# Ankur-Deka/Emergent-Multiagent-Strategies

Measured on AMD Instinct MI355X. Metric: env-steps/sec FortAttack 3v3, 4096 parallel envs per GPU, higher is better.
Workload: dtype f64

## Files before the change

emergent-multiagent-strategies_amd/csrc/fa_collect.hip:

```cpp
#include "fa_device.h"

#define FA_GAE_CHUNK 16
struct FaGaeChunk { float r[FA_GAE_CHUNK], v[FA_GAE_CHUNK], m[FA_GAE_CHUNK]; uint8_t d[FA_GAE_CHUNK]; };
__global__ __launch_bounds__(64) void fa_gae_kernel(const float *__restrict__ rewards,
                                                    const float *__restrict__ value_preds,
                                                    const float *__restrict__ masks,
                                                    float *__restrict__ returns,
                                                    const uint8_t *__restrict__ done, int T, int E,
                                                    int N, float g32, float gt32) {
    const long long EN = (long long)E * N;
    const long long col = (long long)blockIdx.x * blockDim.x + threadIdx.x;
    if (col >= EN) return;
    const int e = (int)(col / N);
    float gae = 0.0f;
    float v_next = value_preds[(long long)T * EN + col];
    float m_next = masks[(long long)T * EN + col];
    auto load = [&](FaGaeChunk &c, int t0) {
#pragma unroll
        for (int k = 0; k < FA_GAE_CHUNK; ++k) {
            const int t = t0 - k;
            const long long o = (long long)(t >= 0 ? t : 0) * EN + col;
            c.r[k] = rewards[o];
            c.v[k] = value_preds[o];
            c.m[k] = masks[o];
            c.d[k] = done[(long long)(t > 0 ? t - 1 : 0) * E + e];
        }
    };
    auto scan = [&](const FaGaeChunk &c, int t0) {
#pragma unroll
        for (int k = 0; k < FA_GAE_CHUNK; ++k) {
            const int t = t0 - k;
            if (t >= 0) {
                const float delta = c.r[k] + g32 * v_next * m_next - c.v[k];
                const float g = delta + gt32 * m_next * gae;
                if ((t > 0) & (c.d[k] != 0)) {
                    gae = 0.0f;
                } else {
                    gae = g;
                    returns[(long long)t * EN + col] = g + c.v[k];
                }
                v_next = c.v[k];
                m_next = c.m[k];
            }
        }
    };
    FaGaeChunk ca, cb;
    load(ca, T - 1);
    for (int t0 = T - 1; t0 >= 0; t0 -= 2 * FA_GAE_CHUNK) {
        load(cb, t0 - FA_GAE_CHUNK);
        scan(ca, t0);
        load(ca, t0 - 2 * FA_GAE_CHUNK);
        scan(cb, t0 - FA_GAE_CHUNK);
    }
}

#define FA_GAEC_CHUNK 32
__global__ __launch_bounds__(256) void fa_gae_coop_kernel(const float *__restrict__ rewards,
                                                          const float *__restrict__ value_preds,
                                                          const float *__restrict__ masks,
                                                          float *__restrict__ returns,
                                                          const uint8_t *__restrict__ done, int T, int E,
                                                          int N, float g32, float gt32) {
    __shared__ float s_r[2][FA_GAEC_CHUNK][64], s_v[2][FA_GAEC_CHUNK][64], s_m[2][FA_GAEC_CHUNK][64];
    __shared__ uint8_t s_d[2][FA_GAEC_CHUNK][64];
    const long long EN = (long long)E * N;
    const int lane = threadIdx.x & 63, wave = threadIdx.x >> 6;
    const long long colv = (long long)blockIdx.x * 64 + lane;
    const bool valid = colv < EN;
    const long long col = valid ? colv : EN - 1;
    const int e = (int)(col / N);
    const int nc = (T + FA_GAEC_CHUNK - 1) / FA_GAEC_CHUNK;
    auto load_chunk = [&](int c) {
        const int t0 = T - 1 - c * FA_GAEC_CHUNK, b = c & 1;
        if (wave == 3) {
            float x[FA_GAEC_CHUNK];
            uint8_t d[FA_GAEC_CHUNK];
#pragma unroll
            for (int k = 0; k < FA_GAEC_CHUNK; ++k) {
                const int t = t0 - k;
                x[k] = masks[(long long)(t >= 0 ? t : 0) * EN + col];
                d[k] = done[(long long)(t > 0 ? t - 1 : 0) * E + e];
            }
#pragma unroll
            for (int k = 0; k < FA_GAEC_CHUNK; ++k) { s_m[b][k][lane] = x[k]; s_d[b][k][lane] = d[k]; }
        } else {
            const float *src = wave == 1 ? rewards : value_preds;
            float x[FA_GAEC_CHUNK];
#pragma unroll
            for (int k = 0; k < FA_GAEC_CHUNK; ++k) {
                const int t = t0 - k;
                x[k] = src[(long long)(t >= 0 ? t : 0) * EN + col];
            }
            float(*dst)[64] = wave == 1 ? s_r[b] : s_v[b];
#pragma unroll
            for (int k = 0; k < FA_GAEC_CHUNK; ++k) dst[k][lane] = x[k];
        }
    };
    float gae = 0.0f, v_next = 0.0f, m_next = 0.0f;
    if (wave == 0) {
        v_next = value_preds[(long long)T * EN + col];
        m_next = masks[(long long)T * EN + col];
    } else {
        load_chunk(0);
    }
    __syncthreads();
    for (int c = 0; c < nc; ++c) {
        if (wave != 0) {
            if (c + 1 < nc) load_chunk(c + 1);
        } else {
            const int t0 = T - 1 - c * FA_GAEC_CHUNK, b = c & 1;
            float r[FA_GAEC_CHUNK], v[FA_GAEC_CHUNK], m[FA_GAEC_CHUNK];
            uint8_t d[FA_GAEC_CHUNK];
#pragma unroll
            for (int k = 0; k < FA_GAEC_CHUNK; ++k) {
                r[k] = s_r[b][k][lane]; v[k] = s_v[b][k][lane]; m[k] = s_m[b][k][lane]; d[k] = s_d[b][k][lane];
            }
#pragma unroll
            for (int k = 0; k < FA_GAEC_CHUNK; ++k) {
                const int t = t0 - k;
                if (t >= 0) {
                    const float delta = r[k] + g32 * v_next * m_next - v[k];
                    const float g = delta + gt32 * m_next * gae;
                    if ((t > 0) & (d[k] != 0)) {
                        gae = 0.0f;
                    } else {
                        gae = g;
                        if (valid) returns[(long long)t * EN + col] = g + v[k];
                    }
                    v_next = v[k];
                    m_next = m[k];
                }
            }
        }
        __syncthreads();
    }
}


#define FA_GAEC_GATHER 4
#define FA_GAEC_BARRIER() asm volatile("s_waitcnt lgkmcnt(0)\n\ts_barrier" ::: "memory")
__device__ __forceinline__ float fa_gae_pivot(const float *__restrict__ rewards, const float *__restrict__ value_preds,
                                              const float *__restrict__ masks, int T, long long EN, int i, float g32) {
    const long long o = (long long)(T - 1) * EN + i, o1 = (long long)T * EN + i;
    const float vp = value_preds[o];
    const float delta = rewards[o] + g32 * value_preds[o1] * masks[o1] - vp;
    return (delta + vp) - vp;
}

__global__ __launch_bounds__(256, 2) void fa_gae_mom_kernel(const float *__restrict__ rewards,
                                                             const float *__restrict__ value_preds,
                                                             const float *__restrict__ masks, float *__restrict__ returns,
                                                             const uint8_t *__restrict__ done, int T, int E, int N, float g32,
                                                             float gt32, double *__restrict__ partial) {
    __shared__ float s_x[3][2][FA_GAEC_CHUNK][64];
    __shared__ uint8_t s_d[2][FA_GAEC_CHUNK][64];
    __shared__ double s_sq[2][64];
    const long long EN = (long long)E * N;
    const int lane = threadIdx.x & 63, wave = __builtin_amdgcn_readfirstlane(threadIdx.x >> 6);
    const long long colv = (long long)blockIdx.x * 64 + lane;
    const bool valid = colv < EN;
    const long long col = valid ? colv : EN - 1;
    const int e = (int)(col / N);
    const int nc = (T + FA_GAEC_CHUNK - 1) / FA_GAEC_CHUNK;
    const unsigned rowb = (unsigned)EN * 4u;
    const unsigned coff = (unsigned)col * 4u;
    const float *src = wave == 1 ? rewards : (wave == 2 ? value_preds : masks);
    const __amdgpu_buffer_rsrc_t rs_src =
        __builtin_amdgcn_make_buffer_rsrc(const_cast<float *>(src), 0, (int)((unsigned)(T + 1) * rowb), 0x00020000);
    const __amdgpu_buffer_rsrc_t rs_ret = __builtin_amdgcn_make_buffer_rsrc(returns, 0, (int)((unsigned)(T + 1) * rowb), 0x00020000);
    const __amdgpu_buffer_rsrc_t rs_val =
        __builtin_amdgcn_make_buffer_rsrc(const_cast<float *>(value_preds), 0, (int)((unsigned)(T + 1) * rowb), 0x00020000);
    const __amdgpu_buffer_rsrc_t rs_done =
        __builtin_amdgcn_make_buffer_rsrc(const_cast<uint8_t *>(done), 0, (int)((unsigned)T * (unsigned)E), 0x00020000);
    auto ldf = [&](const __amdgpu_buffer_rsrc_t &rs, unsigned voff, unsigned soff) -> float {
        return __builtin_bit_cast(float, __builtin_amdgcn_raw_buffer_load_b32(rs, (int)voff, __builtin_amdgcn_readfirstlane((int)soff), 0));
    };
    struct Chunk { float x[FA_GAEC_CHUNK]; uint8_t d[FA_GAEC_CHUNK]; };
    auto issue = [&](Chunk &q, int c) {
        const int t0 = T - 1 - c * FA_GAEC_CHUNK;
#pragma unroll
        for (int k = 0; k < FA_GAEC_CHUNK; ++k) {
            const int t = t0 - k;
            q.x[k] = ldf(rs_src, coff, (unsigned)(t >= 0 ? t : 0) * rowb);
        }
        if (wave == 3) {
#pragma unroll
            for (int k = 0; k < FA_GAEC_CHUNK; ++k) {
                const int t = t0 - k;
                q.d[k] = __builtin_amdgcn_raw_buffer_load_b8(rs_done, e, __builtin_amdgcn_readfirstlane((int)((unsigned)(t > 0 ? t - 1 : 0) * (unsigned)E)), 0);
            }
        }
    };
    auto stash = [&](const Chunk &q, int c) {
        float(*dst)[64] = s_x[wave - 1][c & 1];
#pragma unroll
        for (int k = 0; k < FA_GAEC_CHUNK; ++k) dst[k][lane] = q.x[k];
        if (wave == 3) {
#pragma unroll
            for (int k = 0; k < FA_GAEC_CHUNK; ++k) s_d[c & 1][k][lane] = q.d[k];
        }
    };
    if (wave != 0) {
        Chunk q;
        issue(q, 0);
        stash(q, 0);
        FA_GAEC_BARRIER();
        for (int c = 0; c < nc; ++c) {
            if (c + 1 < nc) {
                issue(q, c + 1);
                stash(q, c + 1);
            }
            FA_GAEC_BARRIER();
        }
    } else {
        float gae = 0.0f;
        float v_next = value_preds[(long long)T * EN + col];
        float m_next = masks[(long long)T * EN + col];
        double accS[2] = {0.0, 0.0}, accQ[2] = {0.0, 0.0};
        const double piv = (double)fa_gae_pivot(rewards, value_preds, masks, T, EN, (int)(col % N), g32);
        auto add_stale = [&](float o, float v) {
            const double dd = (double)(o - v) - piv;
            accS[0] += dd;
            accQ[0] = __fma_rn(dd, dd, accQ[0]);
        };
        float go[FA_GAEC_GATHER], gv[FA_GAEC_GATHER];
        unsigned gmask = 0u;
#pragma unroll
        for (int j = 0; j < FA_GAEC_GATHER; ++j) { go[j] = 0.0f; gv[j] = 0.0f; }
        FA_GAEC_BARRIER();
        auto scan_chunk = [&](int c) {
            const int t0 = T - 1 - c * FA_GAEC_CHUNK, b = c & 1;
#pragma unroll
            for (int j = 0; j < FA_GAEC_GATHER; ++j)
                if ((gmask >> j) & 1u) add_stale(go[j], gv[j]);
            float r[FA_GAEC_CHUNK], v[FA_GAEC_CHUNK], m[FA_GAEC_CHUNK];
            uint8_t d[FA_GAEC_CHUNK];
#pragma unroll
            for (int k = 0; k < FA_GAEC_CHUNK; ++k) {
                r[k] = s_x[0][b][k][lane]; v[k] = s_x[1][b][k][lane]; m[k] = s_x[2][b][k][lane]; d[k] = s_d[b][k][lane];
            }
            unsigned stale = 0u;
#pragma unroll
            for (int k = 0; k < FA_GAEC_CHUNK; ++k) {
                const int t = t0 - k;
                if (t >= 0) {
                    const float delta = r[k] + g32 * v_next * m_next - v[k];
                    const float g = delta + gt32 * m_next * gae;
                    if ((t > 0) & (d[k] != 0)) {
                        gae = 0.0f;
                        stale |= 1u << k;
                    } else {
                        gae = g;
                        const float ret = g + v[k];
                        if (valid) __builtin_amdgcn_raw_buffer_store_b32(__builtin_bit_cast(unsigned, ret), rs_ret, (int)coff, __builtin_amdgcn_readfirstlane((int)((unsigned)t * rowb)), 0);
                        const double dd = (double)(ret - v[k]) - piv;
                        accS[k & 1] += dd;
                        accQ[k & 1] = __fma_rn(dd, dd, accQ[k & 1]);
                    }
                    v_next = v[k];
                    m_next = m[k];
                }
            }
            {
                unsigned rem = stale;
                gmask = 0u;
#pragma unroll
                for (int j = 0; j < FA_GAEC_GATHER; ++j) {
                    const int k = rem ? __builtin_ctz(rem) : 0;
                    gmask |= (rem ? 1u : 0u) << j;
                    rem &= rem - 1u;
                    const unsigned o = (unsigned)(t0 - k) * rowb + coff;
                    go[j] = ldf(rs_ret, o, 0u);
                    gv[j] = ldf(rs_val, o, 0u);
                }
                while (__builtin_amdgcn_ballot_w64(rem != 0u) != 0ull) {
                    const bool has = rem != 0u;
                    const int k = has ? __builtin_ctz(rem) : 0;
                    rem &= rem - 1u;
                    const unsigned o = (unsigned)(t0 - k) * rowb + coff;
                    const float o_ = ldf(rs_ret, o, 0u), v_ = ldf(rs_val, o, 0u);
                    if (has) add_stale(o_, v_);
                }
            }
        };
        for (int c = 0; c < nc; ++c) {
            scan_chunk(c);
            FA_GAEC_BARRIER();
        }
#pragma unroll
        for (int j = 0; j < FA_GAEC_GATHER; ++j)
            if ((gmask >> j) & 1u) add_stale(go[j], gv[j]);
        s_sq[0][lane] = valid ? accS[0] + accS[1] : 0.0;
        s_sq[1][lane] = valid ? accQ[0] + accQ[1] : 0.0;
    }
    {
        __syncthreads();
        if ((int)threadIdx.x < 2 * N) {
            const int i = threadIdx.x >> 1, cmp = threadIdx.x & 1;
            const int first = (int)(((long long)blockIdx.x * 64) % N);
            double acc = 0.0;
            for (int l = (i - first + N) % N; l < 64; l += N) acc += s_sq[cmp][l];
            partial[((long long)blockIdx.x * N + i) * 2 + cmp] = acc;
        }
    }
}

#define FA_GAEM_FOLD 8
__device__ __forceinline__ void fa_gae_mom_fold(const double *__restrict__ partial, int nblocks, int N, int i, int lane,
                                                double n_rows, double piv, double &mean, double &m2) {
    const double2 *p2 = reinterpret_cast<const double2 *>(partial);
    double2 p[FA_GAEM_FOLD];
#pragma unroll
    for (int k = 0; k < FA_GAEM_FOLD; ++k) {
        const int b = lane + 64 * k;
        p[k] = p2[(long long)(b < nblocks ? b : 0) * N + i];
    }
    double s = 0.0, q = 0.0;
#pragma unroll
    for (int k = 0; k < FA_GAEM_FOLD; ++k) {
        const bool in = lane + 64 * k < nblocks;
        s += in ? p[k].x : 0.0;
        q += in ? p[k].y : 0.0;
    }
#pragma unroll
    for (int off = 32; off > 0; off >>= 1) { s += __shfl_down(s, off, 64); q += __shfl_down(q, off, 64); }
    s = __shfl(s, 0, 64);
    q = __shfl(q, 0, 64);
    mean = piv + s / n_rows;
    m2 = q - s * (s / n_rows);
}

__global__ void fa_gae_mom_final_kernel(const double *__restrict__ partial, int nblocks, int N,
                                        const float *__restrict__ rewards, const float *__restrict__ value_preds,
                                        const float *__restrict__ masks, int T, long long EN, float g32, double n_rows,
                                        double *__restrict__ moments_out, double *__restrict__ mean_out,
                                        double *__restrict__ std_out) {
    const int i = threadIdx.x >> 6, lane = threadIdx.x & 63;
    if (i >= N) return;
    const double piv = (double)fa_gae_pivot(rewards, value_preds, masks, T, EN, i, g32);
    double mean, m2;
    fa_gae_mom_fold(partial, nblocks, N, i, lane, n_rows, piv, mean, m2);
    if (lane == 0) {
        if (moments_out) { moments_out[i * 3 + 0] = n_rows; moments_out[i * 3 + 1] = mean; moments_out[i * 3 + 2] = m2; }
        if (mean_out) mean_out[i] = mean;
        if (std_out) std_out[i] = sqrt(m2 / (n_rows - 1.0));
    }
}

__global__ __launch_bounds__(512) void fa_gae_mom_norm_kernel(const double *__restrict__ partial, int nblocks, int N,
                                                              const float *__restrict__ rewards,
                                                              const float *__restrict__ value_preds,
                                                              const float *__restrict__ masks,
                                                              const float *__restrict__ returns, int T, long long EN, float g32,
                                                              double n_rows, long long total, float *__restrict__ out,
                                                              double *__restrict__ moments_out, double *__restrict__ mean_out,
                                                              double *__restrict__ std_out, int piv_from_returns,
                                                              const double *__restrict__ gathered, int W) {
    __shared__ float s_mean[FA_MAX_AGENTS_DEV], s_den[FA_MAX_AGENTS_DEV];
    const int lane = threadIdx.x & 63, wave = threadIdx.x >> 6;
    const long long stride = (long long)gridDim.x * blockDim.x;
    const long long gid = (long long)blockIdx.x * blockDim.x + threadIdx.x;
    const long long quads = total / 4;
    const bool vec = (((uintptr_t)returns | (uintptr_t)value_preds | (uintptr_t)out) & 15) == 0;
    const float4 *r4 = reinterpret_cast<const float4 *>(returns), *v4 = reinterpret_cast<const float4 *>(value_preds);
    float4 ra = make_float4(0.f, 0.f, 0.f, 0.f), va = ra, rb = ra, vb = ra;
    if (vec && gid < quads) {
        const long long q1 = gid + stride;
        ra = r4[gid]; va = v4[gid];
        rb = r4[q1 < quads ? q1 : gid]; vb = v4[q1 < quads ? q1 : gid];
    }
    if (gathered) {
        if ((int)threadIdx.x < N) {
            const int i = threadIdx.x;
            double n = 0.0, mean = 0.0, m2 = 0.0;
            for (int r = 0; r < W; ++r) {
                const double *g = gathered + ((long long)r * N + i) * 3;
                const double nr = g[0], mr = g[1], m2r = g[2];
                if (nr <= 0.0) continue;
                const double nn = n + nr, delta = mr - mean;
                mean += delta * (nr / nn);
                m2 += m2r + delta * delta * (n * nr / nn);
                n = nn;
            }
            const double sd = sqrt(m2 / (n - 1.0));
            s_mean[i] = (float)mean;
            s_den[i] = (float)sd + 1e-5f;
            if (blockIdx.x == 0) {
                if (mean_out) mean_out[i] = mean;
                if (std_out) std_out[i] = sd;
            }
        }
    } else
    for (int i = wave; i < N; i += 8) {
        const double piv = piv_from_returns ? (double)(returns[i] - value_preds[i])
                                            : (double)fa_gae_pivot(rewards, value_preds, masks, T, EN, i, g32);
        double mean, m2;
        fa_gae_mom_fold(partial, nblocks, N, i, lane, n_rows, piv, mean, m2);
        const double sd = sqrt(m2 / (n_rows - 1.0));
        if (lane == 0) {
            s_mean[i] = (float)mean;
            s_den[i] = (float)sd + 1e-5f;
            if (blockIdx.x == 0) {
                if (moments_out) { moments_out[i * 3 + 0] = n_rows; moments_out[i * 3 + 1] = mean; moments_out[i * 3 + 2] = m2; }
                if (mean_out) mean_out[i] = mean;
                if (std_out) std_out[i] = sd;
            }
        }
    }
    __syncthreads();
    if (vec) {
        float4 *o4 = reinterpret_cast<float4 *>(out);
#ifndef FA_NORM_PLAIN_STORES
        typedef int v4i __attribute__((ext_vector_type(4)));
        const bool small = total * 4 < (1LL << 31);
        const __amdgpu_buffer_rsrc_t rs_out = __builtin_amdgcn_make_buffer_rsrc(out, 0, small ? (int)(total * 4) : 0, 0x00020000);
        auto st4 = [&](long long q, const float4 &v) {
            if (small) {
                v4i w = {__builtin_bit_cast(int, v.x), __builtin_bit_cast(int, v.y), __builtin_bit_cast(int, v.z), __builtin_bit_cast(int, v.w)};
                __builtin_amdgcn_raw_buffer_store_b128(w, rs_out, (int)(q * 16), 0, 16);
            } else {
                o4[q] = v;
            }
        };
#else
        auto st4 = [&](long long q, const float4 &v) { o4[q] = v; };
#endif
        for (long long q0 = gid; q0 < quads; q0 += 2 * stride) {
            const long long q1 = q0 + stride;
            const bool two = q1 < quads;
            if (q0 != gid) {
                ra = r4[q0]; va = v4[q0];
                rb = r4[two ? q1 : q0]; vb = v4[two ? q1 : q0];
            }
            auto norm4 = [&](const float4 &r, const float4 &v, long long q) {
                int i = (int)((4 * q) % N);
                float4 o;
                o.x = (r.x - v.x - s_mean[i]) / s_den[i]; i = i + 1 == N ? 0 : i + 1;
                o.y = (r.y - v.y - s_mean[i]) / s_den[i]; i = i + 1 == N ? 0 : i + 1;
                o.z = (r.z - v.z - s_mean[i]) / s_den[i]; i = i + 1 == N ? 0 : i + 1;
                o.w = (r.w - v.w - s_mean[i]) / s_den[i];
                return o;
            };
            st4(q0, norm4(ra, va, q0));
            if (two) st4(q1, norm4(rb, vb, q1));
        }
        for (long long k = quads * 4 + gid; k < total; k += stride) {
            const int i = (int)(k % N);
            out[k] = (returns[k] - value_preds[k] - s_mean[i]) / s_den[i];
        }
    } else {
        for (long long k = gid; k < total; k += stride) {
            const int i = (int)(k % N);
            out[k] = (returns[k] - value_preds[k] - s_mean[i]) / s_den[i];
        }
    }
}

#define FA_GAE4_CHUNK 16
__global__ __launch_bounds__(64) void fa_gae4_kernel(const float *__restrict__ rewards,
                                                     const float *__restrict__ value_preds,
                                                     const float *__restrict__ masks,
                                                     float *__restrict__ returns,
                                                     const uint8_t *__restrict__ done, int T, int E,
                                                     int N, float g32, float gt32) {
    const long long EN = (long long)E * N;
    const long long col = ((long long)blockIdx.x * blockDim.x + threadIdx.x) * 4;
    if (col >= EN) return;
    int e[4];
#pragma unroll
    for (int q = 0; q < 4; ++q) e[q] = (int)((col + q) / N);
    float gae[4] = {0.f, 0.f, 0.f, 0.f};
    float4 v_next = *reinterpret_cast<const float4 *>(value_preds + (long long)T * EN + col);
    float4 m_next = *reinterpret_cast<const float4 *>(masks + (long long)T * EN + col);
    for (int t0 = T - 1; t0 >= 0; t0 -= FA_GAE4_CHUNK) {
        float4 r[FA_GAE4_CHUNK], v[FA_GAE4_CHUNK], m[FA_GAE4_CHUNK];
        unsigned skip[FA_GAE4_CHUNK];
#pragma unroll
        for (int k = 0; k < FA_GAE4_CHUNK; ++k) {
            const int t = t0 - k;
            const bool in = t >= 0;
            const long long o = (long long)(in ? t : 0) * EN + col;
            r[k] = *reinterpret_cast<const float4 *>(rewards + o);
            v[k] = *reinterpret_cast<const float4 *>(value_preds + o);
            m[k] = *reinterpret_cast<const float4 *>(masks + o);
            unsigned sk = 0;
            const uint8_t *d = done + (long long)(t > 0 ? t - 1 : 0) * E;
#pragma unroll
            for (int q = 0; q < 4; ++q) sk |= ((unsigned)(t > 0) & (unsigned)(d[e[q]] != 0)) << q;
            skip[k] = sk;
        }
#pragma unroll
        for (int k = 0; k < FA_GAE4_CHUNK; ++k) {
            const int t = t0 - k;
            if (t >= 0) {
                const float rr[4] = {r[k].x, r[k].y, r[k].z, r[k].w};
                const float vv[4] = {v[k].x, v[k].y, v[k].z, v[k].w};
                const float vn[4] = {v_next.x, v_next.y, v_next.z, v_next.w};
                const float mn[4] = {m_next.x, m_next.y, m_next.z, m_next.w};
                float out[4];
                float *ret = returns + (long long)t * EN + col;
#pragma unroll
                for (int q = 0; q < 4; ++q) {
                    const float delta = rr[q] + g32 * vn[q] * mn[q] - vv[q];
                    const float g = delta + gt32 * mn[q] * gae[q];
                    const bool sk = (skip[k] >> q) & 1u;
                    gae[q] = sk ? 0.0f : g;
                    out[q] = g + vv[q];
                }
                if (skip[k] == 0u) {
                    *reinterpret_cast<float4 *>(ret) = make_float4(out[0], out[1], out[2], out[3]);
                } else {
#pragma unroll
                    for (int q = 0; q < 4; ++q)
                        if (!((skip[k] >> q) & 1u)) ret[q] = out[q];
                }
                v_next = v[k];
                m_next = m[k];
            }
        }
    }
}

template <int PASS>
__global__ __launch_bounds__(256) void fa_adv_partial_kernel(const float *__restrict__ returns,
                                                             const float *__restrict__ value_preds,
                                                             const double *__restrict__ mean, long long rows,
                                                             int N, double *__restrict__ partial) {
    __shared__ double red[4][FA_MAX_AGENTS_DEV];
    double acc[FA_MAX_AGENTS_DEV];
#pragma unroll
    for (int i = 0; i < FA_MAX_AGENTS_DEV; ++i) acc[i] = 0.0;
    double mu[FA_MAX_AGENTS_DEV];
#pragma unroll
    for (int i = 0; i < FA_MAX_AGENTS_DEV; ++i) mu[i] = (PASS == 1 && i < N) ? mean[i] : 0.0;
    const long long stride = (long long)gridDim.x * blockDim.x;
    for (long long r = (long long)blockIdx.x * blockDim.x + threadIdx.x; r < rows; r += stride) {
        const float *ret = returns + r * N, *vp = value_preds + r * N;
#pragma unroll
        for (int i = 0; i < FA_MAX_AGENTS_DEV; ++i) {
            if (i < N) {
                const double adv = (double)(ret[i] - vp[i]);
                if (PASS == 0) acc[i] += adv;
                else { const double d = adv - mu[i]; acc[i] += d * d; }
            }
        }
    }
    const int lane = threadIdx.x & 63, wave = threadIdx.x >> 6;
#pragma unroll
    for (int i = 0; i < FA_MAX_AGENTS_DEV; ++i) {
        double v = acc[i];
#pragma unroll
        for (int off = 32; off > 0; off >>= 1) v += __shfl_down(v, off, 64);
        if (lane == 0) red[wave][i] = v;
    }
    __syncthreads();
    if (threadIdx.x < N) {
        const int i = threadIdx.x;
        partial[((long long)blockIdx.x * N + i)] = ((red[0][i] + red[1][i]) + red[2][i]) + red[3][i];
    }
}

template <int PASS, int TN>
__global__ __launch_bounds__(256) void fa_adv_partial_vec_kernel(const float *__restrict__ returns,
                                                                 const float *__restrict__ value_preds,
                                                                 const double *__restrict__ mean, long long row_pairs,
                                                                 double *__restrict__ partial) {
    constexpr int NV = TN / 2;
    __shared__ double red[4][TN];
    double acc[TN], mu[TN];
#pragma unroll
    for (int i = 0; i < TN; ++i) { acc[i] = 0.0; mu[i] = PASS == 1 ? mean[i] : 0.0; }
    const long long stride = (long long)gridDim.x * blockDim.x;
    for (long long p = (long long)blockIdx.x * blockDim.x + threadIdx.x; p < row_pairs; p += stride) {
        const float4 *r4 = reinterpret_cast<const float4 *>(returns + p * 2 * TN);
        const float4 *v4 = reinterpret_cast<const float4 *>(value_preds + p * 2 * TN);
        float4 rr[NV], vv[NV];
#pragma unroll
        for (int q = 0; q < NV; ++q) { rr[q] = r4[q]; vv[q] = v4[q]; }
#pragma unroll
        for (int q = 0; q < NV; ++q) {
            const float a4[4] = {rr[q].x - vv[q].x, rr[q].y - vv[q].y, rr[q].z - vv[q].z, rr[q].w - vv[q].w};
#pragma unroll
            for (int j = 0; j < 4; ++j) {
                const int i = (4 * q + j) % TN;
                const double adv = (double)a4[j];
                if (PASS == 0) acc[i] += adv;
                else { const double d = adv - mu[i]; acc[i] += d * d; }
            }
        }
    }
    const int lane = threadIdx.x & 63, wave = threadIdx.x >> 6;
#pragma unroll
    for (int i = 0; i < TN; ++i) {
        double v = acc[i];
#pragma unroll
        for (int off = 32; off > 0; off >>= 1) v += __shfl_down(v, off, 64);
        if (lane == 0) red[wave][i] = v;
    }
    __syncthreads();
    if (threadIdx.x < TN) {
        const int i = threadIdx.x;
        partial[((long long)blockIdx.x * TN + i)] = ((red[0][i] + red[1][i]) + red[2][i]) + red[3][i];
    }
}

__device__ __forceinline__ void fa_adv_onepass_finish(double (&acc_s)[FA_MAX_AGENTS_DEV], double (&acc_q)[FA_MAX_AGENTS_DEV],
                                                      int N, double *__restrict__ partial) {
    __shared__ double red[4][FA_MAX_AGENTS_DEV][2];
    const int lane = threadIdx.x & 63, wave = threadIdx.x >> 6;
#pragma unroll
    for (int i = 0; i < FA_MAX_AGENTS_DEV; ++i) {
        if (i < N) {
            double s = acc_s[i], q = acc_q[i];
#pragma unroll
            for (int off = 32; off > 0; off >>= 1) { s += __shfl_down(s, off, 64); q += __shfl_down(q, off, 64); }
            if (lane == 0) { red[wave][i][0] = s; red[wave][i][1] = q; }
        }
    }
    __syncthreads();
    if ((int)threadIdx.x < 2 * N) {
        const int i = threadIdx.x >> 1, c = threadIdx.x & 1;
        partial[((long long)blockIdx.x * N + i) * 2 + c] = ((red[0][i][c] + red[1][i][c]) + red[2][i][c]) + red[3][i][c];
    }
}

#define FA_ADV_FOLD 16
__global__ void fa_adv_onepass_final_kernel(const double *__restrict__ partial, int nblocks, int N,
                                            const float *__restrict__ returns, const float *__restrict__ value_preds,
                                            double n_rows, double *__restrict__ moments_out,
                                            double *__restrict__ mean_out, double *__restrict__ std_out) {
    const int i = threadIdx.x >> 6, lane = threadIdx.x & 63;
    if (i >= N) return;
    double ps[FA_ADV_FOLD], pq[FA_ADV_FOLD];
#pragma unroll
    for (int k = 0; k < FA_ADV_FOLD; ++k) {
        const int b = lane + 64 * k;
        const bool in = b < nblocks;
        const double *p = partial + ((long long)(in ? b : 0) * N + i) * 2;
        ps[k] = in ? p[0] : 0.0;
        pq[k] = in ? p[1] : 0.0;
    }
    double s = 0.0, q = 0.0;
#pragma unroll
    for (int k = 0; k < FA_ADV_FOLD; ++k) { s += ps[k]; q += pq[k]; }
#pragma unroll
    for (int off = 32; off > 0; off >>= 1) { s += __shfl_down(s, off, 64); q += __shfl_down(q, off, 64); }
    if (lane == 0) {
        const double piv = (double)(returns[i] - value_preds[i]);
        const double mean = piv + s / n_rows, m2 = q - s * (s / n_rows);
        if (moments_out) { moments_out[i * 3 + 0] = n_rows; moments_out[i * 3 + 1] = mean; moments_out[i * 3 + 2] = m2; }
        if (mean_out) mean_out[i] = mean;
        if (std_out) std_out[i] = sqrt(m2 / (n_rows - 1.0));
    }
}

__global__ __launch_bounds__(256) void fa_adv_onepass_kernel(const float *__restrict__ returns,
                                                             const float *__restrict__ value_preds, long long rows, int N,
                                                             double *__restrict__ partial) {
    double acc_s[FA_MAX_AGENTS_DEV], acc_q[FA_MAX_AGENTS_DEV], piv[FA_MAX_AGENTS_DEV];
#pragma unroll
    for (int i = 0; i < FA_MAX_AGENTS_DEV; ++i) {
        acc_s[i] = 0.0; acc_q[i] = 0.0;
        piv[i] = i < N ? (double)(returns[i] - value_preds[i]) : 0.0;
    }
    const long long stride = (long long)gridDim.x * blockDim.x;
    for (long long r = (long long)blockIdx.x * blockDim.x + threadIdx.x; r < rows; r += stride) {
        const float *ret = returns + r * N, *vp = value_preds + r * N;
#pragma unroll
        for (int i = 0; i < FA_MAX_AGENTS_DEV; ++i) {
            if (i < N) {
                const double d = (double)(ret[i] - vp[i]) - piv[i];
                acc_s[i] += d;
                acc_q[i] = __fma_rn(d, d, acc_q[i]);
            }
        }
    }
    fa_adv_onepass_finish(acc_s, acc_q, N, partial);
}

template <int TN>
__global__ __launch_bounds__(256) void fa_adv_onepass_vec_kernel(const float *__restrict__ returns,
                                                                 const float *__restrict__ value_preds, long long row_pairs,
                                                                 double *__restrict__ partial) {
    constexpr int NV = TN / 2;
    constexpr int UNR = 4;
    double acc_s[FA_MAX_AGENTS_DEV], acc_q[FA_MAX_AGENTS_DEV], piv[FA_MAX_AGENTS_DEV];
#pragma unroll
    for (int i = 0; i < FA_MAX_AGENTS_DEV; ++i) {
        acc_s[i] = 0.0; acc_q[i] = 0.0;
        piv[i] = i < TN ? (double)(returns[i] - value_preds[i]) : 0.0;
    }
    const long long stride = (long long)gridDim.x * blockDim.x;
    for (long long p0 = (long long)blockIdx.x * blockDim.x + threadIdx.x; p0 < row_pairs; p0 += stride * UNR) {
        float4 rr[UNR][NV], vv[UNR][NV];
#pragma unroll
        for (int u = 0; u < UNR; ++u) {
            const long long p = p0 + u * stride;
            const long long pc = p < row_pairs ? p : p0;
            const float4 *r4 = reinterpret_cast<const float4 *>(returns + pc * 2 * TN);
            const float4 *v4 = reinterpret_cast<const float4 *>(value_preds + pc * 2 * TN);
#pragma unroll
            for (int q = 0; q < NV; ++q) { rr[u][q] = r4[q]; vv[u][q] = v4[q]; }
        }
#pragma unroll
        for (int u = 0; u < UNR; ++u) {
            if (p0 + u * stride < row_pairs) {
#pragma unroll
                for (int q = 0; q < NV; ++q) {
                    const float a4[4] = {rr[u][q].x - vv[u][q].x, rr[u][q].y - vv[u][q].y, rr[u][q].z - vv[u][q].z,
                                         rr[u][q].w - vv[u][q].w};
#pragma unroll
                    for (int j = 0; j < 4; ++j) {
                        const int i = (4 * q + j) % TN;
                        const double d = (double)a4[j] - piv[i];
                        acc_s[i] += d;
                        acc_q[i] = __fma_rn(d, d, acc_q[i]);
                    }
                }
            }
        }
    }
    fa_adv_onepass_finish(acc_s, acc_q, TN, partial);
}

template <int PASS>
__global__ void fa_adv_final_kernel(const double *__restrict__ partial, int nblocks, int N, double n_rows,
                                    double *__restrict__ stats, double *__restrict__ derived) {
    const int i = threadIdx.x >> 6, lane = threadIdx.x & 63;
    if (i >= N) return;
    double s = 0.0;
    for (int b = lane; b < nblocks; b += 64) s += partial[(long long)b * N + i];
#pragma unroll
    for (int off = 32; off > 0; off >>= 1) s += __shfl_down(s, off, 64);
    if (lane == 0) {
        if (PASS == 0) {
            stats[i * 3 + 0] = n_rows; stats[i * 3 + 1] = s; stats[i * 3 + 2] = 0.0;
            if (derived) derived[i] = s / n_rows;
        } else {
            stats[i * 3 + 2] = s;
            if (derived) derived[i] = sqrt(s / (n_rows - 1.0));
        }
    }
}

__global__ __launch_bounds__(256) void fa_adv_norm_kernel(const float *__restrict__ returns,
                                                          const float *__restrict__ value_preds,
                                                          const double *__restrict__ mean,
                                                          const double *__restrict__ std_, long long total,
                                                          int N, float *__restrict__ out) {
    const long long stride = (long long)gridDim.x * blockDim.x;
    for (long long k = (long long)blockIdx.x * blockDim.x + threadIdx.x; k < total; k += stride) {
        const int i = (int)(k % N);
        const float adv = returns[k] - value_preds[k];
        out[k] = (adv - (float)mean[i]) / ((float)std_[i] + 1e-5f);
    }
}

__global__ void fa_adv_merge_kernel(const double *__restrict__ gathered, int W, int N,
                                    double *__restrict__ mean_out, double *__restrict__ std_out) {
    const int i = threadIdx.x;
    if (i >= N) return;
    double n = 0.0, mean = 0.0, m2 = 0.0;
    for (int r = 0; r < W; ++r) {
        const double *g = gathered + ((long long)r * N + i) * 3;
        const double nr = g[0], mr = g[1], m2r = g[2];
        if (nr <= 0.0) continue;
        const double nn = n + nr, delta = mr - mean;
        mean += delta * (nr / nn);
        m2 += m2r + delta * delta * (n * nr / nn);
        n = nn;
    }
    mean_out[i] = mean;
    std_out[i] = sqrt(m2 / (n - 1.0));
}

__global__ void fa_adv_moments_kernel(double *__restrict__ stats, int N) {
    const int i = threadIdx.x;
    if (i >= N) return;
    stats[i * 3 + 1] = stats[i * 3 + 1] / stats[i * 3 + 0];
}

hipError_t fa_launch_adv_merge(const double *gathered, int W, int N, double *mean_out, double *std_out,
                               hipStream_t st) {
    hipLaunchKernelGGL(fa_adv_merge_kernel, dim3(1), dim3(64), 0, st, gathered, W, N, mean_out, std_out);
    return hipGetLastError();
}
hipError_t fa_launch_adv_moments_fix(double *stats, int N, hipStream_t st) {
    hipLaunchKernelGGL(fa_adv_moments_kernel, dim3(1), dim3(64), 0, st, stats, N);
    return hipGetLastError();
}

hipError_t fa_launch_gae(const float *rewards, const float *value_preds, const float *masks, float *returns,
                         const uint8_t *done, int T, int E, int N, double gamma, double tau, hipStream_t st) {
    const long long EN = (long long)E * N;
    const bool vec4 = (EN >= 4LL * 64 * 1024) && (EN % 4 == 0) && ((((uintptr_t)rewards | (uintptr_t)value_preds | (uintptr_t)masks |
                                          (uintptr_t)returns) & 15) == 0);
    if (!vec4 && EN <= 64LL * 2048) {
        const int grid = (int)((EN + 63) / 64);
        hipLaunchKernelGGL(fa_gae_coop_kernel, dim3(grid), dim3(256), 0, st, rewards, value_preds, masks, returns,
                           done, T, E, N, (float)gamma, (float)(gamma * tau));
        return hipGetLastError();
    }
    if (vec4) {
        const int grid = (int)((EN / 4 + 63) / 64);
        hipLaunchKernelGGL(fa_gae4_kernel, dim3(grid), dim3(64), 0, st, rewards, value_preds, masks, returns,
                           done, T, E, N, (float)gamma, (float)(gamma * tau));
    } else {
        const int grid = (int)((EN + 63) / 64);
        hipLaunchKernelGGL(fa_gae_kernel, dim3(grid), dim3(64), 0, st, rewards, value_preds, masks, returns,
                           done, T, E, N, (float)gamma, (float)(gamma * tau));
    }
    return hipGetLastError();
}

int fa_gae_mom_blocks(const float *rewards, const float *value_preds, const float *masks, const float *returns, int T, int E,
                      int N, long long partial_cap) {
    const long long EN = (long long)E * N;
    if (EN > 64LL * 512 || T < 1 || (long long)(T + 1) * EN * 4 >= (1LL << 31)) return 0;
    const long long nb = (EN + 63) / 64;
    if (nb > 64 * FA_GAEM_FOLD || nb * N * 2 > partial_cap) return 0;
    return (int)nb;
}
hipError_t fa_launch_gae_mom(const float *rewards, const float *value_preds, const float *masks, float *returns,
                             const uint8_t *done, int T, int E, int N, double gamma, double tau, double *partial, int nblocks,
                             hipStream_t st) {
    hipLaunchKernelGGL(fa_gae_mom_kernel, dim3(nblocks), dim3(256), 0, st, rewards, value_preds, masks, returns, done, T, E, N,
                       (float)gamma, (float)(gamma * tau), partial);
    return hipGetLastError();
}
hipError_t fa_launch_gae_mom_final(const double *partial, int nblocks, const float *rewards, const float *value_preds,
                                   const float *masks, int T, int E, int N, double gamma, double *moments_out, double *mean_out,
                                   double *std_out, hipStream_t st) {
    const long long EN = (long long)E * N;
    const double n_rows = (double)T * (double)E;
    hipLaunchKernelGGL(fa_gae_mom_final_kernel, dim3(1), dim3(64 * N), 0, st, partial, nblocks, N, rewards, value_preds, masks, T,
                       EN, (float)gamma, n_rows, moments_out, mean_out, std_out);
    return hipGetLastError();
}
hipError_t fa_launch_gae_mom_norm(const double *partial, int nblocks, const float *rewards, const float *value_preds,
                                  const float *masks, const float *returns, int T, int E, int N, double gamma, float *out,
                                  double *moments_out, double *mean_out, double *std_out, int grid, int piv_from_returns,
                                  hipStream_t st) {
    const long long EN = (long long)E * N, total = (long long)T * EN;
    const double n_rows = (double)T * (double)E;
    if (grid <= 0) {
        long long want = (total / 4 + 1023) / 1024;
        grid = (int)(want < 512 ? (want < 1 ? 1 : want) : 512);
    }
    hipLaunchKernelGGL(fa_gae_mom_norm_kernel, dim3(grid), dim3(512), 0, st, partial, nblocks, N, rewards, value_preds, masks,
                       returns, T, EN, (float)gamma, n_rows, total, out, moments_out, mean_out, std_out, piv_from_returns,
                       (const double *)nullptr, 0);
    return hipGetLastError();
}
hipError_t fa_launch_adv_merge_norm(const double *gathered, int W, int N, const float *returns, const float *value_preds,
                                    long long total, float *out, double *mean_out, double *std_out, hipStream_t st) {
    long long want = (total / 4 + 1023) / 1024;
    const int grid = (int)(want < 512 ? (want < 1 ? 1 : want) : 512);
    hipLaunchKernelGGL(fa_gae_mom_norm_kernel, dim3(grid), dim3(512), 0, st, (const double *)nullptr, 0, N, (const float *)nullptr,
                       value_preds, (const float *)nullptr, returns, 0, 0LL, 0.0f, 0.0, total, out, (double *)nullptr, mean_out,
                       std_out, 0, gathered, W);
    return hipGetLastError();
}

hipError_t fa_launch_adv_onepass(const float *returns, const float *value_preds, long long rows, int N, double *partial,
                                 int nblocks, double *moments_out, double *mean_out, double *std_out, hipStream_t st,
                                 bool final = true) {
    const bool vec = (rows % 2 == 0) && ((((uintptr_t)returns | (uintptr_t)value_preds) & 15) == 0);
    if (nblocks > 64 * FA_ADV_FOLD) nblocks = 64 * FA_ADV_FOLD;
    if (vec && N == 6)
        hipLaunchKernelGGL((fa_adv_onepass_vec_kernel<6>), dim3(nblocks), dim3(256), 0, st, returns, value_preds, rows / 2,
                           partial);
    else if (vec && N == 10)
        hipLaunchKernelGGL((fa_adv_onepass_vec_kernel<10>), dim3(nblocks), dim3(256), 0, st, returns, value_preds, rows / 2,
                           partial);
    else
        hipLaunchKernelGGL(fa_adv_onepass_kernel, dim3(nblocks), dim3(256), 0, st, returns, value_preds, rows, N, partial);
    if (final)
        hipLaunchKernelGGL(fa_adv_onepass_final_kernel, dim3(1), dim3(64 * N), 0, st, partial, nblocks, N, returns, value_preds,
                           (double)rows, moments_out, mean_out, std_out);
    return hipGetLastError();
}

template <int PASS>
static void launch_adv_partial(const float *returns, const float *value_preds, const double *mean, long long rows,
                               int N, double *partial, int nblocks, hipStream_t st) {
    const bool vec = (rows % 2 == 0) && ((((uintptr_t)returns | (uintptr_t)value_preds) & 15) == 0);
    if (vec && N == 6)
        hipLaunchKernelGGL((fa_adv_partial_vec_kernel<PASS, 6>), dim3(nblocks), dim3(256), 0, st, returns, value_preds,
                           mean, rows / 2, partial);
    else if (vec && N == 10)
        hipLaunchKernelGGL((fa_adv_partial_vec_kernel<PASS, 10>), dim3(nblocks), dim3(256), 0, st, returns, value_preds,
                           mean, rows / 2, partial);
    else
        hipLaunchKernelGGL(fa_adv_partial_kernel<PASS>, dim3(nblocks), dim3(256), 0, st, returns, value_preds, mean,
                           rows, N, partial);
}

hipError_t fa_launch_adv_stats(int pass, const float *returns, const float *value_preds, const double *mean,
                               long long rows, int N, double *partial, int nblocks, double *stats,
                               double *derived, hipStream_t st) {
    if (pass == 0) {
        launch_adv_partial<0>(returns, value_preds, mean, rows, N, partial, nblocks, st);
        hipLaunchKernelGGL(fa_adv_final_kernel<0>, dim3(1), dim3(64 * N), 0, st, partial, nblocks, N,
                           (double)rows, stats, derived);
    } else {
        launch_adv_partial<1>(returns, value_preds, mean, rows, N, partial, nblocks, st);
        hipLaunchKernelGGL(fa_adv_final_kernel<1>, dim3(1), dim3(64 * N), 0, st, partial, nblocks, N,
                           (double)rows, stats, derived);
    }
    return hipGetLastError();
}

hipError_t fa_launch_adv_norm(const float *returns, const float *value_preds, const double *mean,
                              const double *std_, long long total, int N, float *out, hipStream_t st) {
    long long want = (total + 255) / 256;
    const int grid = (int)(want < 2048 ? (want < 1 ? 1 : want) : 2048);
    hipLaunchKernelGGL(fa_adv_norm_kernel, dim3(grid), dim3(256), 0, st, returns, value_preds, mean, std_,
                       total, N, out);
    return hipGetLastError();
}
```

Before: 3.131 billion.

## Split GAE-moment kernel into loader, scan, store and moment wave stages

Restructures the fused GAE+moments kernel into a three-stage software pipeline across eight waves. Three loader waves each precompute delta, the decay coefficient and flags for a slice of every chunk. One wave runs only the serial gae recurrence. Two waves write returns, and two parity waves accumulate the mean and variance moments and gather stale entries. The aim is to take delta arithmetic, stores and double-precision moment work off the serial scan's critical path. In exchange it uses more threads and shared memory (triple buffering), adds one extra barrier trip, and drops the occupancy hint of 2 blocks.

```diff
diff --git a/emergent-multiagent-strategies_amd/csrc/fa_collect.hip b/emergent-multiagent-strategies_amd/csrc/fa_collect.hip
--- a/emergent-multiagent-strategies_amd/csrc/fa_collect.hip
+++ b/emergent-multiagent-strategies_amd/csrc/fa_collect.hip
@@ -147,14 +147,45 @@
     return (delta + vp) - vp;
 }
 
-__global__ __launch_bounds__(256, 2) void fa_gae_mom_kernel(const float *__restrict__ rewards,
-                                                             const float *__restrict__ value_preds,
-                                                             const float *__restrict__ masks, float *__restrict__ returns,
-                                                             const uint8_t *__restrict__ done, int T, int E, int N, float g32,
-                                                             float gt32, double *__restrict__ partial) {
-    __shared__ float s_x[3][2][FA_GAEC_CHUNK][64];
-    __shared__ uint8_t s_d[2][FA_GAEC_CHUNK][64];
-    __shared__ double s_sq[2][64];
+#define FA_GAES_LOADERS 3
+#define FA_GAES_THREADS (64 * (FA_GAES_LOADERS + 5))
+#define FA_GAES_LIVE 0
+#define FA_GAES_STALE 1
+#define FA_GAES_BELOW 2
+constexpr int fa_gaes_first(int l) { return (l * FA_GAEC_CHUNK + FA_GAES_LOADERS - 1) / FA_GAES_LOADERS; }
+constexpr bool fa_gaes_one_owner_per_step() {
+    for (int k = 0; k < FA_GAEC_CHUNK; ++k) {
+        int owners = 0;
+        for (int l = 0; l < FA_GAES_LOADERS; ++l) owners += (k >= fa_gaes_first(l) && k < fa_gaes_first(l + 1)) ? 1 : 0;
+        if (owners != 1) return false;
+    }
+    return true;
+}
+constexpr int fa_gaes_max_requests() {
+    int most = 0;
+    for (int l = 0; l < FA_GAES_LOADERS; ++l) {
+        const int n = fa_gaes_first(l + 1) - fa_gaes_first(l);
+        most = 4 * n + 2 > most ? 4 * n + 2 : most;
+    }
+    return most;
+}
+static_assert(fa_gaes_one_owner_per_step(), "every step of a chunk has exactly one loader");
+static_assert(fa_gaes_max_requests() <= 63, "a wave has at most 63 vector-memory requests in flight (vmcnt)");
+__device__ __forceinline__ int fa_gaes_trips(int nc) { return nc + 2; }
+__device__ __forceinline__ int fa_gaes_load_chunk(int j, int nc) { return j < nc ? j : -1; }
+__device__ __forceinline__ int fa_gaes_scan_chunk(int j, int nc) { return (j >= 1 && j - 1 < nc) ? j - 1 : -1; }
+__device__ __forceinline__ int fa_gaes_post_chunk(int j, int nc) { return (j >= 2 && j - 2 < nc) ? j - 2 : -1; }
+template <int L> struct FaGaesLoader { static constexpr int first = fa_gaes_first(L), n = fa_gaes_first(L + 1) - fa_gaes_first(L); };
+template <int P> struct FaGaesParity { static constexpr int value = P; };
+
+__global__ __launch_bounds__(FA_GAES_THREADS) void fa_gae_mom_kernel(const float *__restrict__ rewards,
+                                                                     const float *__restrict__ value_preds,
+                                                                     const float *__restrict__ masks, float *__restrict__ returns,
+                                                                     const uint8_t *__restrict__ done, int T, int E, int N, float g32,
+                                                                     float gt32, double *__restrict__ partial) {
+    __shared__ float s_g[3][FA_GAEC_CHUNK][64], s_v[3][FA_GAEC_CHUNK][64], s_c[2][FA_GAEC_CHUNK][64];
+    __shared__ uint8_t s_f[3][FA_GAEC_CHUNK][64];
+    __shared__ double s_sq[2][2][64];
     const long long EN = (long long)E * N;
     const int lane = threadIdx.x & 63, wave = __builtin_amdgcn_readfirstlane(threadIdx.x >> 6);
     const long long colv = (long long)blockIdx.x * 64 + lane;
@@ -162,136 +193,172 @@
     const long long col = valid ? colv : EN - 1;
     const int e = (int)(col / N);
     const int nc = (T + FA_GAEC_CHUNK - 1) / FA_GAEC_CHUNK;
+    const int trips = fa_gaes_trips(nc);
     const unsigned rowb = (unsigned)EN * 4u;
     const unsigned coff = (unsigned)col * 4u;
-    const float *src = wave == 1 ? rewards : (wave == 2 ? value_preds : masks);
-    const __amdgpu_buffer_rsrc_t rs_src =
-        __builtin_amdgcn_make_buffer_rsrc(const_cast<float *>(src), 0, (int)((unsigned)(T + 1) * rowb), 0x00020000);
-    const __amdgpu_buffer_rsrc_t rs_ret = __builtin_amdgcn_make_buffer_rsrc(returns, 0, (int)((unsigned)(T + 1) * rowb), 0x00020000);
-    const __amdgpu_buffer_rsrc_t rs_val =
-        __builtin_amdgcn_make_buffer_rsrc(const_cast<float *>(value_preds), 0, (int)((unsigned)(T + 1) * rowb), 0x00020000);
-    const __amdgpu_buffer_rsrc_t rs_done =
-        __builtin_amdgcn_make_buffer_rsrc(const_cast<uint8_t *>(done), 0, (int)((unsigned)T * (unsigned)E), 0x00020000);
+    auto rsrc = [&](const void *p, unsigned bytes) {
+        return __builtin_amdgcn_make_buffer_rsrc(const_cast<void *>(p), 0, (int)bytes, 0x00020000);
+    };
+    const __amdgpu_buffer_rsrc_t rs_rew = rsrc(rewards, (unsigned)T * rowb);
+    const __amdgpu_buffer_rsrc_t rs_val = rsrc(value_preds, (unsigned)(T + 1) * rowb);
+    const __amdgpu_buffer_rsrc_t rs_msk = rsrc(masks, (unsigned)(T + 1) * rowb);
+    const __amdgpu_buffer_rsrc_t rs_ret = rsrc(returns, (unsigned)(T + 1) * rowb);
+    const __amdgpu_buffer_rsrc_t rs_done = rsrc(done, (unsigned)T * (unsigned)E);
     auto ldf = [&](const __amdgpu_buffer_rsrc_t &rs, unsigned voff, unsigned soff) -> float {
         return __builtin_bit_cast(float, __builtin_amdgcn_raw_buffer_load_b32(rs, (int)voff, __builtin_amdgcn_readfirstlane((int)soff), 0));
     };
-    struct Chunk { float x[FA_GAEC_CHUNK]; uint8_t d[FA_GAEC_CHUNK]; };
-    auto issue = [&](Chunk &q, int c) {
-        const int t0 = T - 1 - c * FA_GAEC_CHUNK;
-#pragma unroll
-        for (int k = 0; k < FA_GAEC_CHUNK; ++k) {
-            const int t = t0 - k;
-            q.x[k] = ldf(rs_src, coff, (unsigned)(t >= 0 ? t : 0) * rowb);
-        }
-        if (wave == 3) {
-#pragma unroll
-            for (int k = 0; k < FA_GAEC_CHUNK; ++k) {
-                const int t = t0 - k;
-                q.d[k] = __builtin_amdgcn_raw_buffer_load_b8(rs_done, e, __builtin_amdgcn_readfirstlane((int)((unsigned)(t > 0 ? t - 1 : 0) * (unsigned)E)), 0);
-            }
-        }
-    };
-    auto stash = [&](const Chunk &q, int c) {
-        float(*dst)[64] = s_x[wave - 1][c & 1];
-#pragma unroll
-        for (int k = 0; k < FA_GAEC_CHUNK; ++k) dst[k][lane] = q.x[k];
-        if (wave == 3) {
-#pragma unroll
-            for (int k = 0; k < FA_GAEC_CHUNK; ++k) s_d[c & 1][k][lane] = q.d[k];
-        }
-    };
-    if (wave != 0) {
-        Chunk q;
-        issue(q, 0);
-        stash(q, 0);
-        FA_GAEC_BARRIER();
-        for (int c = 0; c < nc; ++c) {
-            if (c + 1 < nc) {
-                issue(q, c + 1);
-                stash(q, c + 1);
+    if (wave >= 1 && wave <= FA_GAES_LOADERS) {
+        auto load_chunk = [&](auto who, int c) {
+            constexpr int k0 = decltype(who)::first, n = decltype(who)::n;
+            const int t0 = T - 1 - c * FA_GAEC_CHUNK - k0;
+            float v[n + 1], m[n + 1], r[n];
+            uint8_t d[n];
+#pragma unroll
+            for (int i = 0; i <= n; ++i) {
+                const int t = t0 + 1 - i;
+                const unsigned so = (unsigned)(t >= 0 ? t : 0) * rowb;
+                v[i] = ldf(rs_val, coff, so);
+                m[i] = ldf(rs_msk, coff, so);
+                if (i < n) {
+                    r[i] = ldf(rs_rew, coff, (unsigned)(t >= 1 ? t - 1 : 0) * rowb);
+                    d[i] = __builtin_amdgcn_raw_buffer_load_b8(rs_done, e, __builtin_amdgcn_readfirstlane((int)((unsigned)(t >= 2 ? t - 2 : 0) * (unsigned)E)), 0);
+                }
+            }
+            const int b3 = c % 3, b2 = c & 1;
+#pragma unroll
+            for (int i = 0; i < n; ++i) {
+                const int t = t0 - i;
+                const float delta = r[i] + g32 * v[i] * m[i] - v[i + 1];
+                s_g[b3][k0 + i][lane] = delta;
+                s_c[b2][k0 + i][lane] = gt32 * m[i];
+                s_v[b3][k0 + i][lane] = v[i + 1];
+                s_f[b3][k0 + i][lane] = t < 0 ? FA_GAES_BELOW : (((t > 0) & (d[i] != 0)) ? FA_GAES_STALE : FA_GAES_LIVE);
+            }
+        };
+        auto run = [&](auto who) {
+            for (int j = 0; j < trips; ++j) {
+                const int c = fa_gaes_load_chunk(j, nc);
+                if (c >= 0) load_chunk(who, c);
+                FA_GAEC_BARRIER();
+            }
+        };
+        static_assert(FA_GAES_LOADERS == 3, "one branch per loader below");
+        if (wave == 1) run(FaGaesLoader<0>());
+        else if (wave == 2) run(FaGaesLoader<1>());
+        else run(FaGaesLoader<2>());
+    } else if (wave == 0) {
+        float gae = 0.0f;
+        for (int j = 0; j < trips; ++j) {
+            const int c = fa_gaes_scan_chunk(j, nc);
+            if (c >= 0) {
+                const int b3 = c % 3, b2 = c & 1;
+                float dl[FA_GAEC_CHUNK], cc[FA_GAEC_CHUNK];
+                uint8_t f[FA_GAEC_CHUNK];
+#pragma unroll
+                for (int k = 0; k < FA_GAEC_CHUNK; ++k) { dl[k] = s_g[b3][k][lane]; cc[k] = s_c[b2][k][lane]; f[k] = s_f[b3][k][lane]; }
+#pragma unroll
+                for (int k = 0; k < FA_GAEC_CHUNK; ++k) {
+                    const float g = dl[k] + cc[k] * gae;
+                    s_g[b3][k][lane] = g;
+                    gae = f[k] != FA_GAES_LIVE ? 0.0f : g;
+                }
             }
             FA_GAEC_BARRIER();
         }
+    } else if (wave < FA_GAES_LOADERS + 3) {
+        const int par = wave - (FA_GAES_LOADERS + 1);
+        for (int j = 0; j < trips; ++j) {
+            const int c = fa_gaes_post_chunk(j, nc);
+            if (c >= 0) {
+                const int t0 = T - 1 - c * FA_GAEC_CHUNK - par, b3 = c % 3;
+                float g[FA_GAEC_CHUNK / 2], v[FA_GAEC_CHUNK / 2];
+                uint8_t f[FA_GAEC_CHUNK / 2];
+#pragma unroll
+                for (int i = 0; i < FA_GAEC_CHUNK / 2; ++i) {
+                    g[i] = s_g[b3][2 * i + par][lane]; v[i] = s_v[b3][2 * i + par][lane]; f[i] = s_f[b3][2 * i + par][lane];
+                }
+#pragma unroll
+                for (int i = 0; i < FA_GAEC_CHUNK / 2; ++i) {
+                    const int t = t0 - 2 * i;
+                    const float ret = g[i] + v[i];
+                    if (valid & (f[i] == FA_GAES_LIVE)) __builtin_amdgcn_raw_buffer_store_b32(__builtin_bit_cast(unsigned, ret), rs_ret, (int)coff, __builtin_amdgcn_readfirstlane((int)((unsigned)t * rowb)), 0);
+                }
+            }
+            FA_GAEC_BARRIER();
+        }
     } else {
-        float gae = 0.0f;
-        float v_next = value_preds[(long long)T * EN + col];
-        float m_next = masks[(long long)T * EN + col];
-        double accS[2] = {0.0, 0.0}, accQ[2] = {0.0, 0.0};
-        const double piv = (double)fa_gae_pivot(rewards, value_preds, masks, T, EN, (int)(col % N), g32);
-        auto add_stale = [&](float o, float v) {
-            const double dd = (double)(o - v) - piv;
-            accS[0] += dd;
-            accQ[0] = __fma_rn(dd, dd, accQ[0]);
+        auto run = [&](auto parity) {
+            constexpr int par = decltype(parity)::value;
+            double accS = 0.0, accQ = 0.0;
+            const double piv = (double)fa_gae_pivot(rewards, value_preds, masks, T, EN, (int)(col % N), g32);
+            auto add_stale = [&](float o, float v) {
+                const double dd = (double)(o - v) - piv;
+                accS += dd;
+                accQ = __fma_rn(dd, dd, accQ);
+            };
+            float go[FA_GAEC_GATHER], gv[FA_GAEC_GATHER];
+            unsigned gmask = 0u;
+#pragma unroll
+            for (int j = 0; j < FA_GAEC_GATHER; ++j) { go[j] = 0.0f; gv[j] = 0.0f; }
+            for (int j = 0; j < trips; ++j) {
+                const int c = fa_gaes_post_chunk(j, nc);
+                if (c >= 0) {
+                    const int t0 = T - 1 - c * FA_GAEC_CHUNK, b3 = c % 3;
+                    if (par == 0) {
+#pragma unroll
+                        for (int q = 0; q < FA_GAEC_GATHER; ++q)
+                            if ((gmask >> q) & 1u) add_stale(go[q], gv[q]);
+                    }
+                    float g[FA_GAEC_CHUNK / 2], v[FA_GAEC_CHUNK / 2];
+                    uint8_t f[FA_GAEC_CHUNK];
+#pragma unroll
+                    for (int i = 0; i < FA_GAEC_CHUNK / 2; ++i) { g[i] = s_g[b3][2 * i + par][lane]; v[i] = s_v[b3][2 * i + par][lane]; }
+#pragma unroll
+                    for (int k = 0; k < FA_GAEC_CHUNK; ++k) f[k] = (par == 0 || (k & 1) == par) ? s_f[b3][k][lane] : 0;
+#pragma unroll
+                    for (int i = 0; i < FA_GAEC_CHUNK / 2; ++i) {
+                        const float ret = g[i] + v[i];
+                        const double d0 = (double)(ret - v[i]) - piv;
+                        const double dd = f[2 * i + par] == FA_GAES_LIVE ? d0 : 0.0;
+                        accS += dd;
+                        accQ = __fma_rn(dd, dd, accQ);
+                    }
+                    if (par == 0) {
+                        unsigned rem = 0u;
+#pragma unroll
+                        for (int k = 0; k < FA_GAEC_CHUNK; ++k) rem |= (f[k] == FA_GAES_STALE ? 1u : 0u) << k;
+                        gmask = 0u;
+#pragma unroll
+                        for (int q = 0; q < FA_GAEC_GATHER; ++q) {
+                            const int k = rem ? __builtin_ctz(rem) : 0;
+                            gmask |= (rem ? 1u : 0u) << q;
+                            rem &= rem - 1u;
+                            const unsigned o = (unsigned)(t0 - k) * rowb + coff;
+                            go[q] = ldf(rs_ret, o, 0u);
+                            gv[q] = ldf(rs_val, o, 0u);
+                        }
+                        while (__builtin_amdgcn_ballot_w64(rem != 0u) != 0ull) {
+                            const bool has = rem != 0u;
+                            const int k = has ? __builtin_ctz(rem) : 0;
+                            rem &= rem - 1u;
+                            const unsigned o = (unsigned)(t0 - k) * rowb + coff;
+                            const float o_ = ldf(rs_ret, o, 0u), v_ = ldf(rs_val, o, 0u);
+                            if (has) add_stale(o_, v_);
+                        }
+                    }
+                }
+                FA_GAEC_BARRIER();
+            }
+            if (par == 0) {
+#pragma unroll
+                for (int q = 0; q < FA_GAEC_GATHER; ++q)
+                    if ((gmask >> q) & 1u) add_stale(go[q], gv[q]);
+            }
+            s_sq[par][0][lane] = valid ? accS : 0.0;
+            s_sq[par][1][lane] = valid ? accQ : 0.0;
         };
-        float go[FA_GAEC_GATHER], gv[FA_GAEC_GATHER];
-        unsigned gmask = 0u;
-#pragma unroll
-        for (int j = 0; j < FA_GAEC_GATHER; ++j) { go[j] = 0.0f; gv[j] = 0.0f; }
-        FA_GAEC_BARRIER();
-        auto scan_chunk = [&](int c) {
-            const int t0 = T - 1 - c * FA_GAEC_CHUNK, b = c & 1;
-#pragma unroll
-            for (int j = 0; j < FA_GAEC_GATHER; ++j)
-                if ((gmask >> j) & 1u) add_stale(go[j], gv[j]);
-            float r[FA_GAEC_CHUNK], v[FA_GAEC_CHUNK], m[FA_GAEC_CHUNK];
-            uint8_t d[FA_GAEC_CHUNK];
-#pragma unroll
-            for (int k = 0; k < FA_GAEC_CHUNK; ++k) {
-                r[k] = s_x[0][b][k][lane]; v[k] = s_x[1][b][k][lane]; m[k] = s_x[2][b][k][lane]; d[k] = s_d[b][k][lane];
-            }
-            unsigned stale = 0u;
-#pragma unroll
-            for (int k = 0; k < FA_GAEC_CHUNK; ++k) {
-                const int t = t0 - k;
-                if (t >= 0) {
-                    const float delta = r[k] + g32 * v_next * m_next - v[k];
-                    const float g = delta + gt32 * m_next * gae;
-                    if ((t > 0) & (d[k] != 0)) {
-                        gae = 0.0f;
-                        stale |= 1u << k;
-                    } else {
-                        gae = g;
-                        const float ret = g + v[k];
-                        if (valid) __builtin_amdgcn_raw_buffer_store_b32(__builtin_bit_cast(unsigned, ret), rs_ret, (int)coff, __builtin_amdgcn_readfirstlane((int)((unsigned)t * rowb)), 0);
-                        const double dd = (double)(ret - v[k]) - piv;
-                        accS[k & 1] += dd;
-                        accQ[k & 1] = __fma_rn(dd, dd, accQ[k & 1]);
-                    }
-                    v_next = v[k];
-                    m_next = m[k];
-                }
-            }
-            {
-                unsigned rem = stale;
-                gmask = 0u;
-#pragma unroll
-                for (int j = 0; j < FA_GAEC_GATHER; ++j) {
-                    const int k = rem ? __builtin_ctz(rem) : 0;
-                    gmask |= (rem ? 1u : 0u) << j;
-                    rem &= rem - 1u;
-                    const unsigned o = (unsigned)(t0 - k) * rowb + coff;
-                    go[j] = ldf(rs_ret, o, 0u);
-                    gv[j] = ldf(rs_val, o, 0u);
-                }
-                while (__builtin_amdgcn_ballot_w64(rem != 0u) != 0ull) {
-                    const bool has = rem != 0u;
-                    const int k = has ? __builtin_ctz(rem) : 0;
-                    rem &= rem - 1u;
-                    const unsigned o = (unsigned)(t0 - k) * rowb + coff;
-                    const float o_ = ldf(rs_ret, o, 0u), v_ = ldf(rs_val, o, 0u);
-                    if (has) add_stale(o_, v_);
-                }
-            }
-        };
-        for (int c = 0; c < nc; ++c) {
-            scan_chunk(c);
-            FA_GAEC_BARRIER();
-        }
-#pragma unroll
-        for (int j = 0; j < FA_GAEC_GATHER; ++j)
-            if ((gmask >> j) & 1u) add_stale(go[j], gv[j]);
-        s_sq[0][lane] = valid ? accS[0] + accS[1] : 0.0;
-        s_sq[1][lane] = valid ? accQ[0] + accQ[1] : 0.0;
+        if (wave == FA_GAES_LOADERS + 3) run(FaGaesParity<0>());
+        else run(FaGaesParity<1>());
     }
     {
         __syncthreads();
@@ -299,7 +366,7 @@
             const int i = threadIdx.x >> 1, cmp = threadIdx.x & 1;
             const int first = (int)(((long long)blockIdx.x * 64) % N);
             double acc = 0.0;
-            for (int l = (i - first + N) % N; l < 64; l += N) acc += s_sq[cmp][l];
+            for (int l = (i - first + N) % N; l < 64; l += N) acc += s_sq[0][cmp][l] + s_sq[1][cmp][l];
             partial[((long long)blockIdx.x * N + i) * 2 + cmp] = acc;
         }
     }
@@ -824,7 +891,7 @@
 hipError_t fa_launch_gae_mom(const float *rewards, const float *value_preds, const float *masks, float *returns,
                              const uint8_t *done, int T, int E, int N, double gamma, double tau, double *partial, int nblocks,
                              hipStream_t st) {
-    hipLaunchKernelGGL(fa_gae_mom_kernel, dim3(nblocks), dim3(256), 0, st, rewards, value_preds, masks, returns, done, T, E, N,
+    hipLaunchKernelGGL(fa_gae_mom_kernel, dim3(nblocks), dim3(FA_GAES_THREADS), 0, st, rewards, value_preds, masks, returns, done, T, E, N,
                        (float)gamma, (float)(gamma * tau), partial);
     return hipGetLastError();
 }
```

After: 3.253 billion (median of 6 runs). 1.04x the previous value.
